# PKU-Alignment/SafeVLA

Measured on AMD Instinct MI355X. Metric: env-steps/sec through PPO-Lagrangian update, higher is better.
Workload: dtype bf16

## Files before the change

### safevla_amd/csrc/attn_q1.hip

```cpp
#include "attn_common.h"

#define Q1_D 512
#define Q1_H 8
#define Q1_WAVES 8
#define Q1_THREADS (Q1_WAVES * 64)
#define Q1_SMAX 256
#define Q1_SLOTS (Q1_SMAX / Q1_WAVES)
#define Q1_RED_FLOATS (Q1_H * Q1_D)
#define Q1_LDS_FWD ((size_t)(Q1_SMAX * Q1_H + 4 * Q1_RED_FLOATS) * sizeof(float))
#define Q1_LDS_BWD ((size_t)(2 * Q1_SMAX * Q1_H + 4 * Q1_RED_FLOATS) * sizeof(float))

__device__ __forceinline__ void q1_unpack(bf16x8 v, float (&f)[8]) {
    const u32x4 w = __builtin_bit_cast(u32x4, v);
#pragma unroll
    for (int i = 0; i < 4; ++i) { f[2 * i] = bf_lo(w[i]); f[2 * i + 1] = bf_hi(w[i]); }
}

__device__ __forceinline__ void q1_token_head_products(const bf16_t* __restrict__ X, const bf16_t* __restrict__ V, int S, float mul, float* out, int w, int lane) {
    constexpr int NT = Q1_SMAX / (16 * Q1_WAVES), NK = Q1_D / 32;
    const int ql = lane & 15, g = lane >> 4;
    const bf16_t* vb = V + (size_t)(ql & (Q1_H - 1)) * Q1_D + 8 * g;
    bf16x8 a[NT][NK], b[NK];
#pragma unroll
    for (int tt = 0; tt < NT; ++tt) {
        const bf16_t* xa = X + (size_t)min((w + Q1_WAVES * tt) * 16 + ql, S - 1) * Q1_D + 8 * g;
#pragma unroll
        for (int kk = 0; kk < NK; ++kk) a[tt][kk] = *(const bf16x8*)(xa + kk * 32);
    }
#pragma unroll
    for (int kk = 0; kk < NK; ++kk) b[kk] = *(const bf16x8*)(vb + kk * 32);
#pragma unroll
    for (int tt = 0; tt < NT; ++tt) {
        const int j0 = (w + Q1_WAVES * tt) * 16;
        f32x4 acc = {0.f, 0.f, 0.f, 0.f};
#pragma unroll
        for (int kk = 0; kk < NK; ++kk) acc = mfma16(a[tt][kk], b[kk], acc);
        if (ql < Q1_H) {
#pragma unroll
            for (int i = 0; i < 4; ++i) {
                const int j = j0 + 4 * g + i;
                if (j < S) out[j * Q1_H + ql] = acc[i] * mul;
            }
        }
    }
}

__device__ __forceinline__ void q1_load_slices(const bf16_t* __restrict__ X, int S, int w, int lane, bf16x8 (&xr)[Q1_SLOTS]) {
#pragma unroll
    for (int t = 0; t < Q1_SLOTS; ++t) {
        const int j = min(w + Q1_WAVES * t, S - 1);
        xr[t] = *(const bf16x8*)(X + (size_t)j * Q1_D + lane * 8);
    }
}

__device__ __forceinline__ void q1_token_sums(const bf16x8 (&xr)[Q1_SLOTS], const float* coef, int S, int w, float (&acc)[Q1_H][8]) {
#pragma unroll
    for (int h = 0; h < Q1_H; ++h)
#pragma unroll
        for (int e = 0; e < 8; ++e) acc[h][e] = 0.f;
#pragma unroll
    for (int t = 0; t < Q1_SLOTS; ++t) {
        const int j = w + Q1_WAVES * t;
        if (j < S) {
            const f32x4 c0 = *(const f32x4*)(coef + j * Q1_H), c1 = *(const f32x4*)(coef + j * Q1_H + 4);
            float x[8];
            q1_unpack(xr[t], x);
#pragma unroll
            for (int h = 0; h < 4; ++h)
#pragma unroll
                for (int e = 0; e < 8; ++e) { acc[h][e] += c0[h] * x[e]; acc[h + 4][e] += c1[h] * x[e]; }
        }
    }
}

__device__ __forceinline__ void q1_red_store(const float (&acc)[Q1_H][8], float* buf, int lane) {
#pragma unroll
    for (int h = 0; h < Q1_H; ++h) {
        *(f32x4*)(buf + h * Q1_D + lane * 8) = f32x4{acc[h][0], acc[h][1], acc[h][2], acc[h][3]};
        *(f32x4*)(buf + h * Q1_D + lane * 8 + 4) = f32x4{acc[h][4], acc[h][5], acc[h][6], acc[h][7]};
    }
}
__device__ __forceinline__ void q1_red_add(float (&acc)[Q1_H][8], const float* buf, int lane) {
#pragma unroll
    for (int h = 0; h < Q1_H; ++h) {
        const f32x4 a = *(const f32x4*)(buf + h * Q1_D + lane * 8), b = *(const f32x4*)(buf + h * Q1_D + lane * 8 + 4);
#pragma unroll
        for (int e = 0; e < 4; ++e) { acc[h][e] += a[e]; acc[h][e + 4] += b[e]; }
    }
}
__device__ __forceinline__ void q1_reduce_write(float (&acc)[Q1_H][8], float* red, int w, int lane, bf16_t* __restrict__ out) {
    if (w >= 4) q1_red_store(acc, red + (w - 4) * Q1_RED_FLOATS, lane);
    __syncthreads();
    if (w < 4) q1_red_add(acc, red + w * Q1_RED_FLOATS, lane);
    if (w == 2 || w == 3) q1_red_store(acc, red + w * Q1_RED_FLOATS, lane);
    __syncthreads();
    if (w < 2) q1_red_add(acc, red + (w + 2) * Q1_RED_FLOATS, lane);
    if (w == 1) q1_red_store(acc, red + Q1_RED_FLOATS, lane);
    __syncthreads();
    if (w == 0) {
        q1_red_add(acc, red + Q1_RED_FLOATS, lane);
#pragma unroll
        for (int h = 0; h < Q1_H; ++h) *(bf16x8*)(out + h * Q1_D + lane * 8) = pack8(acc[h]);
    }
}

struct Q1Args {
    const bf16_t* X; long ldx;
    const bf16_t* QT;
    bf16_t* C; float* SIG; float* P;
    const bf16_t* DC; const float* DSIG;
    bf16_t* DX; long lddx; bf16_t* DQT;
    int S; float scale; DropCfg drop;
};

__global__ void __launch_bounds__(Q1_THREADS, 1) attn_q1_fwd_kernel(Q1Args p) {
    extern __shared__ __attribute__((aligned(16))) char smem[];
    float* sc = (float*)smem;
    float* red = sc + Q1_SMAX * Q1_H;
    const int w = __builtin_amdgcn_readfirstlane(threadIdx.x >> 6), lane = threadIdx.x & 63, S = p.S;
    const size_t r = blockIdx.x;
    const DropCfg drop = drop_resolve(p.drop);
    const bf16_t* X = p.X + r * p.ldx;
    q1_token_head_products(X, p.QT + r * (Q1_H * Q1_D), S, p.scale, sc, w, lane);
    bf16x8 xr[Q1_SLOTS];
    q1_load_slices(X, S, w, lane, xr);
    __syncthreads();
    {
        const int h = w;
        float v[Q1_SMAX / 64], m = -INFINITY, sum = 0.f, sig = 0.f;
#pragma unroll
        for (int i = 0; i < Q1_SMAX / 64; ++i) {
            const int j = lane + 64 * i;
            v[i] = j < S ? sc[j * Q1_H + h] : -INFINITY;
            m = fmaxf(m, v[i]);
        }
        m = wave_max(m);
#pragma unroll
        for (int i = 0; i < Q1_SMAX / 64; ++i) { v[i] = __expf(v[i] - m); sum += v[i]; }
        const float inv = 1.f / wave_sum(sum);
        const unsigned long long e0 = att_drop_row(S, Q1_H, (int)r, h, 0);
#pragma unroll
        for (int i = 0; i < Q1_SMAX / 64; ++i) {
            const int j = lane + 64 * i;
            if (j < S) {
                const float pr = v[i] * inv;
                const float pd = (!drop.thr || att_keep1(drop, e0 + j)) ? pr * drop.scale : 0.f;
                p.P[(r * Q1_H + h) * S + j] = pr;
                sc[j * Q1_H + h] = pd;
                sig += pd;
            }
        }
        sig = wave_sum(sig);
        if (lane == 0) p.SIG[r * Q1_H + h] = sig;
    }
    __syncthreads();
    float acc[Q1_H][8];
    q1_token_sums(xr, sc, S, w, acc);
    q1_reduce_write(acc, red, w, lane, p.C + r * (Q1_H * Q1_D));
}

__global__ void __launch_bounds__(Q1_THREADS, 1) attn_q1_bwd_kernel(Q1Args p) {
    extern __shared__ __attribute__((aligned(16))) char smem[];
    float* dsb = (float*)smem;
    float* pdb = dsb + Q1_SMAX * Q1_H;
    float* red = pdb + Q1_SMAX * Q1_H;
    const int w = __builtin_amdgcn_readfirstlane(threadIdx.x >> 6), lane = threadIdx.x & 63, S = p.S;
    const size_t r = blockIdx.x;
    const DropCfg drop = drop_resolve(p.drop);
    const bf16_t* X = p.X + r * p.ldx;
    q1_token_head_products(X, p.DC + r * (Q1_H * Q1_D), S, 1.f, dsb, w, lane);
    bf16x8 xr[Q1_SLOTS];
    q1_load_slices(X, S, w, lane, xr);
    __syncthreads();
    {
        const int h = w;
        const float dsig = p.DSIG[r * Q1_H + h];
        const unsigned long long e0 = att_drop_row(S, Q1_H, (int)r, h, 0);
        float pr[Q1_SMAX / 64], dp[Q1_SMAX / 64], delta = 0.f;
#pragma unroll
        for (int i = 0; i < Q1_SMAX / 64; ++i) {
            const int j = lane + 64 * i;
            pr[i] = 0.f; dp[i] = 0.f;
            if (j < S) {
                pr[i] = p.P[(r * Q1_H + h) * S + j];
                const bool keep = !drop.thr || att_keep1(drop, e0 + j);
                dp[i] = keep ? (dsb[j * Q1_H + h] + dsig) * drop.scale : 0.f;
                pdb[j * Q1_H + h] = keep ? pr[i] * drop.scale : 0.f;
                delta += pr[i] * dp[i];
            }
        }
        delta = wave_sum(delta);
#pragma unroll
        for (int i = 0; i < Q1_SMAX / 64; ++i) {
            const int j = lane + 64 * i;
            if (j < S) dsb[j * Q1_H + h] = p.scale * pr[i] * (dp[i] - delta);
        }
    }
    __syncthreads();
    {
        float acc[Q1_H][8];
        q1_token_sums(xr, dsb, S, w, acc);
        q1_reduce_write(acc, red, w, lane, p.DQT + r * (Q1_H * Q1_D));
    }
    float qf[Q1_H][8], cf[Q1_H][8];
    const bf16_t* QT = p.QT + r * (Q1_H * Q1_D) + lane * 8;
    const bf16_t* DC = p.DC + r * (Q1_H * Q1_D) + lane * 8;
#pragma unroll
    for (int h = 0; h < Q1_H; ++h) {
        q1_unpack(*(const bf16x8*)(QT + h * Q1_D), qf[h]);
        q1_unpack(*(const bf16x8*)(DC + h * Q1_D), cf[h]);
    }
    bf16_t* DX = p.DX + r * p.lddx;
#pragma unroll 1
    for (int j = w; j < S; j += Q1_WAVES) {
        const f32x4 s0 = *(const f32x4*)(dsb + j * Q1_H), s1 = *(const f32x4*)(dsb + j * Q1_H + 4);
        const f32x4 d0 = *(const f32x4*)(pdb + j * Q1_H), d1 = *(const f32x4*)(pdb + j * Q1_H + 4);
        float o[8];
#pragma unroll
        for (int e = 0; e < 8; ++e) o[e] = 0.f;
#pragma unroll
        for (int h = 0; h < 4; ++h)
#pragma unroll
            for (int e = 0; e < 8; ++e) {
                o[e] += s0[h] * qf[h][e] + d0[h] * cf[h][e];
                o[e] += s1[h] * qf[h + 4][e] + d1[h] * cf[h + 4][e];
            }
        *(bf16x8*)(DX + (size_t)j * Q1_D + lane * 8) = pack8(o);
    }
}

static bool q1_shape_ok(int R, int S, long ldx) { return R > 0 && S > 0 && S <= Q1_SMAX && ldx >= (long)S * Q1_D && ldx % 8 == 0; }

extern "C" int svla_attn_q1_fwd_bf16(const bf16_t* X, long ldx, const bf16_t* QT, bf16_t* C, float* SIG, float* P, int R, int S, float scale,
                                     const svla_dropout* drop, void* stream) {
    if (!X || !QT || !C || !SIG || !P || !q1_shape_ok(R, S, ldx)) return SVLA_EINVAL;
    Q1Args p{};
    p.X = X; p.ldx = ldx; p.QT = QT; p.C = C; p.SIG = SIG; p.P = P; p.S = S; p.scale = scale; p.drop = drop_cfg(drop);
    return svla_launch<attn_q1_fwd_kernel>(dim3(R), dim3(Q1_THREADS), Q1_LDS_FWD, (hipStream_t)stream, p);
}

extern "C" int svla_attn_q1_bwd_bf16(const bf16_t* X, long ldx, const bf16_t* QT, const bf16_t* DC, const float* DSIG, const float* P,
                                     bf16_t* DX, long lddx, bf16_t* DQT, int R, int S, float scale, const svla_dropout* drop, void* stream) {
    if (!X || !QT || !DC || !DSIG || !P || !DX || !DQT || !q1_shape_ok(R, S, ldx) || !q1_shape_ok(R, S, lddx)) return SVLA_EINVAL;
    Q1Args p{};
    p.X = X; p.ldx = ldx; p.QT = QT; p.DC = DC; p.DSIG = DSIG; p.P = (float*)P; p.DX = DX; p.lddx = lddx; p.DQT = DQT;
    p.S = S; p.scale = scale; p.drop = drop_cfg(drop);
    return svla_launch<attn_q1_bwd_kernel>(dim3(R), dim3(Q1_THREADS), Q1_LDS_BWD, (hipStream_t)stream, p);
}

__global__ void __launch_bounds__(256) head_expand_kernel(const bf16_t* __restrict__ v, long ldv, int R, bf16_t* __restrict__ E, const float* __restrict__ bias,
                                                          float* __restrict__ dot, const float* __restrict__ sigma, bf16_t* __restrict__ vs) {
    const size_t r = (size_t)blockIdx.x * 4 + (threadIdx.x >> 6);
    const int lane = threadIdx.x & 63, hl = lane >> 3;
    if (r >= (size_t)R) return;
    const bf16x8 x = *(const bf16x8*)(v + r * ldv + lane * 8);
    const bf16x8 z = {0, 0, 0, 0, 0, 0, 0, 0};
#pragma unroll
    for (int h = 0; h < Q1_H; ++h) *(bf16x8*)(E + (r * Q1_H + h) * Q1_D + lane * 8) = h == hl ? x : z;
    if (!bias && !sigma) return;
    float f[8];
    q1_unpack(x, f);
    if (bias) {
        float s = 0.f;
#pragma unroll
        for (int e = 0; e < 8; ++e) s += f[e] * bias[lane * 8 + e];
        s += __shfl_xor(s, 1, 64); s += __shfl_xor(s, 2, 64); s += __shfl_xor(s, 4, 64);
        if ((lane & 7) == 0) dot[r * Q1_H + hl] = s;
    }
    if (sigma) {
        const float sg = sigma[r * Q1_H + hl];
#pragma unroll
        for (int e = 0; e < 8; ++e) f[e] *= sg;
        *(bf16x8*)(vs + r * Q1_D + lane * 8) = pack8(f);
    }
}
__global__ void __launch_bounds__(256) head_pick_kernel(const bf16_t* __restrict__ G, int R, const float* __restrict__ sigma, const float* __restrict__ bias,
                                                        bf16_t* __restrict__ out, long ldo) {
    const size_t r = (size_t)blockIdx.x * 4 + (threadIdx.x >> 6);
    const int lane = threadIdx.x & 63, hl = lane >> 3;
    if (r >= (size_t)R) return;
    bf16x8 x = *(const bf16x8*)(G + (r * Q1_H + hl) * Q1_D + lane * 8);
    if (sigma) {
        float f[8];
        q1_unpack(x, f);
        const float sg = sigma[r * Q1_H + hl];
#pragma unroll
        for (int e = 0; e < 8; ++e) f[e] += sg * bias[lane * 8 + e];
        x = pack8(f);
    }
    *(bf16x8*)(out + r * ldo + lane * 8) = x;
}

extern "C" int svla_head_expand_bf16(const bf16_t* v, long ldv, int R, bf16_t* E, const float* bias, float* dot, const float* sigma, bf16_t* vs, void* stream) {
    if (!v || !E || R <= 0 || ldv < Q1_D || ldv % 8 || (bias && !dot) || (sigma && !vs)) return SVLA_EINVAL;
    hipLaunchKernelGGL(head_expand_kernel, dim3((R + 3) / 4), dim3(256), 0, (hipStream_t)stream, v, ldv, R, E, bias, dot, sigma, vs);
    return svla_launch_status();
}
extern "C" int svla_head_pick_bf16(const bf16_t* G, int R, const float* sigma, const float* bias, bf16_t* out, long ldo, void* stream) {
    if (!G || !out || R <= 0 || ldo < Q1_D || ldo % 8 || (sigma && !bias)) return SVLA_EINVAL;
    hipLaunchKernelGGL(head_pick_kernel, dim3((R + 3) / 4), dim3(256), 0, (hipStream_t)stream, G, R, sigma, bias, out, ldo);
    return svla_launch_status();
}
```

Measured before the change: 8030.

## Add persistent register-resident streaming kernels for single-query attention fwd/bwd

Adds new persistent forward and backward kernels for single-query cross-attention, made the default path; the old two-pass kernels stay behind an environment variable. Each workgroup holds a row's tokens in registers, computes scores with MFMA from a swizzled LDS image, and prefetches the next row's X, QT and DC while finishing the current row. Grid size is capped at the CU count. The aim is to read X once per row instead of twice and to hide global load latency. In exchange it uses heavy register and LDS pressure at one workgroup per CU, and occupancy is lower.

```diff
diff --git a/safevla_amd/csrc/attn_q1.hip b/safevla_amd/csrc/attn_q1.hip
--- a/safevla_amd/csrc/attn_q1.hip
+++ b/safevla_amd/csrc/attn_q1.hip
@@ -1,3 +1,4 @@
+#include <stdlib.h>
 #include "attn_common.h"
 
 #define Q1_D 512
@@ -231,9 +232,18 @@
 
 static bool q1_shape_ok(int R, int S, long ldx) { return R > 0 && S > 0 && S <= Q1_SMAX && ldx >= (long)S * Q1_D && ldx % 8 == 0; }
 
+int svla_q1_stream_fwd(const bf16_t* X, long ldx, const bf16_t* QT, bf16_t* C, float* SIG, float* P, int R, int S, float scale, DropCfg drop, hipStream_t stream);
+int svla_q1_stream_bwd(const bf16_t* X, long ldx, const bf16_t* QT, const bf16_t* DC, const float* DSIG, const float* P, bf16_t* DX, long lddx, bf16_t* DQT,
+                       int R, int S, float scale, DropCfg drop, hipStream_t stream);
+static bool q1_two_pass() {
+    static const bool on = [] { const char* e = getenv("SVLA_Q1_TWO_PASS"); return e && *e && strcmp(e, "0") != 0; }();
+    return on;
+}
+
 extern "C" int svla_attn_q1_fwd_bf16(const bf16_t* X, long ldx, const bf16_t* QT, bf16_t* C, float* SIG, float* P, int R, int S, float scale,
                                      const svla_dropout* drop, void* stream) {
     if (!X || !QT || !C || !SIG || !P || !q1_shape_ok(R, S, ldx)) return SVLA_EINVAL;
+    if (!q1_two_pass()) return svla_q1_stream_fwd(X, ldx, QT, C, SIG, P, R, S, scale, drop_cfg(drop), (hipStream_t)stream);
     Q1Args p{};
     p.X = X; p.ldx = ldx; p.QT = QT; p.C = C; p.SIG = SIG; p.P = P; p.S = S; p.scale = scale; p.drop = drop_cfg(drop);
     return svla_launch<attn_q1_fwd_kernel>(dim3(R), dim3(Q1_THREADS), Q1_LDS_FWD, (hipStream_t)stream, p);
@@ -242,6 +252,7 @@
 extern "C" int svla_attn_q1_bwd_bf16(const bf16_t* X, long ldx, const bf16_t* QT, const bf16_t* DC, const float* DSIG, const float* P,
                                      bf16_t* DX, long lddx, bf16_t* DQT, int R, int S, float scale, const svla_dropout* drop, void* stream) {
     if (!X || !QT || !DC || !DSIG || !P || !DX || !DQT || !q1_shape_ok(R, S, ldx) || !q1_shape_ok(R, S, lddx)) return SVLA_EINVAL;
+    if (!q1_two_pass()) return svla_q1_stream_bwd(X, ldx, QT, DC, DSIG, P, DX, lddx, DQT, R, S, scale, drop_cfg(drop), (hipStream_t)stream);
     Q1Args p{};
     p.X = X; p.ldx = ldx; p.QT = QT; p.DC = DC; p.DSIG = DSIG; p.P = (float*)P; p.DX = DX; p.lddx = lddx; p.DQT = DQT;
     p.S = S; p.scale = scale; p.drop = drop_cfg(drop);
diff --git a/safevla_amd/csrc/attn_q1_stream.hip b/safevla_amd/csrc/attn_q1_stream.hip
--- /dev/null
+++ b/safevla_amd/csrc/attn_q1_stream.hip
@@ -0,0 +1,301 @@
+#include "attn_common.h"
+
+#define QS_D 512
+#define QS_H 8
+#define QS_WAVES 8
+#define QS_THREADS (QS_WAVES * 64)
+#define QS_SMAX 256
+#define QS_SLOTS (QS_SMAX / QS_WAVES)
+#define QS_TILE_ELEMS (16 * QS_D)
+#define QS_STAGE_BYTES ((size_t)QS_WAVES * QS_TILE_ELEMS * sizeof(bf16_t))
+#define QS_RED_FLOATS (QS_H * QS_D)
+#define QS_COEF_FLOATS (QS_SMAX * QS_H)
+#define QS_VTAB_BYTES ((size_t)QS_H * QS_D * sizeof(bf16_t))
+#define QS_LDS_FWD (QS_STAGE_BYTES + (size_t)QS_COEF_FLOATS * sizeof(float) + QS_VTAB_BYTES)
+#define QS_LDS_BWD (QS_STAGE_BYTES + (size_t)2 * QS_COEF_FLOATS * sizeof(float) + 2 * QS_VTAB_BYTES)
+static_assert(QS_WAVES * QS_RED_FLOATS * sizeof(float) <= QS_STAGE_BYTES, "the 8 partials alias the staging images");
+static_assert(QS_LDS_BWD <= 160 * 1024, "one workgroup's LDS");
+
+struct Q1SArgs {
+    const bf16_t* X; long ldx;
+    const bf16_t* QT;
+    bf16_t* C; float* SIG; float* P;
+    const bf16_t* DC; const float* DSIG;
+    bf16_t* DX; long lddx; bf16_t* DQT;
+    int R, S; float scale; DropCfg drop;
+};
+
+#define QS_FRESH(w_, lane_, S_) asm volatile("" : "+s"(w_), "+v"(lane_), "+s"(S_))
+
+__device__ __forceinline__ void qs_unpack(bf16x8 v, float (&f)[8]) {
+    const u32x4 w = __builtin_bit_cast(u32x4, v);
+#pragma unroll
+    for (int i = 0; i < 4; ++i) { f[2 * i] = bf_lo(w[i]); f[2 * i + 1] = bf_hi(w[i]); }
+}
+
+__device__ __forceinline__ int qs_tile0(int w, int tt) { return (w + QS_WAVES * tt) * 16; }
+
+__device__ __forceinline__ void qs_load_row(const bf16_t* __restrict__ X, int S, int w, int lane, bf16x8 (&xr)[QS_SLOTS]) {
+#pragma unroll
+    for (int t = 0; t < QS_SLOTS; ++t) {
+        const int j = min(qs_tile0(w, t >> 4) + (t & 15), S - 1);
+        xr[t] = *(const bf16x8*)(X + (size_t)j * QS_D + lane * 8);
+    }
+}
+__device__ __forceinline__ void qs_vtab_put(bf16_t* vtab, int w, int lane, bf16x8 v) {
+    asm volatile("" : "+s"(w), "+v"(lane));
+    *(bf16x8*)(vtab + w * QS_D + ((lane ^ (2 * w)) << 3)) = v;
+}
+
+template <int TT> __device__ __forceinline__ void qs_tile_products(const bf16x8 (&xr)[QS_SLOTS], const bf16_t* vtab, bf16_t* img, int S, float mul, float* out,
+                                                                   int w, int lane) {
+    const int ql = lane & 15, g = lane >> 4, hh = lane & (QS_H - 1);
+#pragma unroll
+    for (int i = 0; i < 16; ++i) *(bf16x8*)(img + i * QS_D + ((lane ^ i) << 3)) = xr[16 * TT + i];
+    f32x4 acc = {0.f, 0.f, 0.f, 0.f};
+#pragma unroll
+    for (int kk = 0; kk < QS_D / 32; ++kk)
+        acc = mfma16(*(const bf16x8*)(img + ql * QS_D + (((4 * kk + g) ^ ql) << 3)), *(const bf16x8*)(vtab + hh * QS_D + (((4 * kk + g) ^ (2 * hh)) << 3)), acc);
+    if (ql < QS_H) {
+#pragma unroll
+        for (int i = 0; i < 4; ++i) {
+            const int j = qs_tile0(w, TT) + 4 * g + i;
+            if (j < S) out[j * QS_H + ql] = acc[i] * mul;
+        }
+    }
+}
+__device__ __forceinline__ void qs_products(const bf16x8 (&xr)[QS_SLOTS], const bf16_t* vtab, bf16_t* img, int S, float mul, float* out, int w, int lane) {
+    QS_FRESH(w, lane, S);
+    if (qs_tile0(w, 0) < S) qs_tile_products<0>(xr, vtab, img, S, mul, out, w, lane);
+    if (qs_tile0(w, 1) < S) qs_tile_products<1>(xr, vtab, img, S, mul, out, w, lane);
+}
+
+__device__ __forceinline__ void qs_token_sums_refill(bf16x8 (&xr)[QS_SLOTS], const float* coef, int S, int w, int lane, const bf16_t* __restrict__ Xn,
+                                                     float (&acc)[QS_H][8]) {
+    QS_FRESH(w, lane, S);
+#pragma unroll
+    for (int h = 0; h < QS_H; ++h)
+#pragma unroll
+        for (int e = 0; e < 8; ++e) acc[h][e] = 0.f;
+#pragma unroll
+    for (int t = 0; t < QS_SLOTS; ++t) {
+        const int j = qs_tile0(w, t >> 4) + (t & 15);
+        if (j < S) {
+            const f32x4 c0 = *(const f32x4*)(coef + j * QS_H), c1 = *(const f32x4*)(coef + j * QS_H + 4);
+            float x[8];
+            qs_unpack(xr[t], x);
+#pragma unroll
+            for (int h = 0; h < 4; ++h)
+#pragma unroll
+                for (int e = 0; e < 8; ++e) { acc[h][e] += c0[h] * x[e]; acc[h + 4][e] += c1[h] * x[e]; }
+        }
+        xr[t] = *(const bf16x8*)(Xn + (size_t)min(j, S - 1) * QS_D + lane * 8);
+    }
+}
+
+__device__ __forceinline__ void qs_red_put(const float (&acc)[QS_H][8], float* red, int w, int lane) {
+    asm volatile("" : "+s"(w), "+v"(lane));
+#pragma unroll
+    for (int h = 0; h < QS_H; ++h) {
+        *(f32x4*)(red + w * QS_RED_FLOATS + h * QS_D + lane * 4) = f32x4{acc[h][0], acc[h][1], acc[h][2], acc[h][3]};
+        *(f32x4*)(red + w * QS_RED_FLOATS + h * QS_D + 256 + lane * 4) = f32x4{acc[h][4], acc[h][5], acc[h][6], acc[h][7]};
+    }
+}
+__device__ __forceinline__ void qs_head_sum_write(const float* red, int w, int lane, bf16_t* __restrict__ out) {
+    asm volatile("" : "+s"(w), "+v"(lane));
+    float s[8] = {0.f, 0.f, 0.f, 0.f, 0.f, 0.f, 0.f, 0.f};
+#pragma unroll
+    for (int v = 0; v < QS_WAVES; ++v) {
+        const f32x4 a = *(const f32x4*)(red + v * QS_RED_FLOATS + w * QS_D + lane * 4), b = *(const f32x4*)(red + v * QS_RED_FLOATS + w * QS_D + 256 + lane * 4);
+#pragma unroll
+        for (int e = 0; e < 4; ++e) { s[e] += a[e]; s[e + 4] += b[e]; }
+    }
+    *(bf16x8*)(out + w * QS_D + lane * 8) = pack8(s);
+}
+
+__global__ void __launch_bounds__(QS_THREADS, 1) attn_q1_stream_fwd_kernel(Q1SArgs p) {
+    extern __shared__ __attribute__((aligned(16))) char smem[];
+    bf16_t* stage = (bf16_t*)smem;
+    float* red = (float*)smem;
+    float* sc = (float*)(smem + QS_STAGE_BYTES);
+    bf16_t* vtab = (bf16_t*)(sc + QS_COEF_FLOATS);
+    const int w = __builtin_amdgcn_readfirstlane(threadIdx.x >> 6), lane = threadIdx.x & 63, S = p.S;
+    const DropCfg drop = drop_resolve(p.drop);
+    bf16_t* img = stage + w * QS_TILE_ELEMS;
+    size_t r = blockIdx.x;
+    bf16x8 xr[QS_SLOTS];
+    qs_load_row(p.X + r * p.ldx, S, w, lane, xr);
+    qs_vtab_put(vtab, w, lane, *(const bf16x8*)(p.QT + r * (QS_H * QS_D) + threadIdx.x * 8));
+    __syncthreads();
+    for (;;) {
+        const size_t rn = r + gridDim.x;
+        const bool more = rn < (size_t)p.R;
+        const size_t rl = more ? rn : r;
+        int tid = threadIdx.x;
+        asm volatile("" : "+v"(tid));
+        const bf16x8 vq = *(const bf16x8*)(p.QT + rl * (QS_H * QS_D) + tid * 8);
+        qs_products(xr, vtab, img, S, p.scale, sc, w, lane);
+        __syncthreads();
+        qs_vtab_put(vtab, w, lane, vq);
+        {
+            const int h = w;
+            float v[QS_SMAX / 64], m = -INFINITY, sum = 0.f, sig = 0.f;
+#pragma unroll
+            for (int i = 0; i < QS_SMAX / 64; ++i) {
+                const int j = lane + 64 * i;
+                v[i] = j < S ? sc[j * QS_H + h] : -INFINITY;
+                m = fmaxf(m, v[i]);
+            }
+            m = wave_max(m);
+#pragma unroll
+            for (int i = 0; i < QS_SMAX / 64; ++i) { v[i] = __expf(v[i] - m); sum += v[i]; }
+            const float inv = 1.f / wave_sum(sum);
+            const unsigned long long e0 = att_drop_row(S, QS_H, (int)r, h, 0);
+#pragma unroll
+            for (int i = 0; i < QS_SMAX / 64; ++i) {
+                const int j = lane + 64 * i;
+                if (j < S) {
+                    const float pr = v[i] * inv;
+                    const float pd = (!drop.thr || att_keep1(drop, e0 + j)) ? pr * drop.scale : 0.f;
+                    p.P[(r * QS_H + h) * S + j] = pr;
+                    sc[j * QS_H + h] = pd;
+                    sig += pd;
+                }
+            }
+            sig = wave_sum(sig);
+            if (lane == 0) p.SIG[r * QS_H + h] = sig;
+        }
+        __syncthreads();
+        float acc[QS_H][8];
+        qs_token_sums_refill(xr, sc, S, w, lane, p.X + rl * p.ldx, acc);
+        qs_red_put(acc, red, w, lane);
+        __syncthreads();
+        qs_head_sum_write(red, w, lane, p.C + r * (QS_H * QS_D));
+        if (!more) break;
+        r = rn;
+        __syncthreads();
+    }
+}
+
+__global__ void __launch_bounds__(QS_THREADS, 1) attn_q1_stream_bwd_kernel(Q1SArgs p) {
+    extern __shared__ __attribute__((aligned(16))) char smem[];
+    bf16_t* stage = (bf16_t*)smem;
+    float* red = (float*)smem;
+    float* dsb = (float*)(smem + QS_STAGE_BYTES);
+    float* pdb = dsb + QS_COEF_FLOATS;
+    bf16_t* vdc = (bf16_t*)(pdb + QS_COEF_FLOATS);
+    bf16_t* vqt = vdc + QS_H * QS_D;
+    const int w = __builtin_amdgcn_readfirstlane(threadIdx.x >> 6), lane = threadIdx.x & 63, S = p.S;
+    const DropCfg drop = drop_resolve(p.drop);
+    bf16_t* img = stage + w * QS_TILE_ELEMS;
+    size_t r = blockIdx.x;
+    bf16x8 xr[QS_SLOTS];
+    qs_load_row(p.X + r * p.ldx, S, w, lane, xr);
+    float pr[QS_SMAX / 64], dsig;
+#pragma unroll
+    for (int i = 0; i < QS_SMAX / 64; ++i) {
+        const int j = lane + 64 * i;
+        pr[i] = p.P[(r * QS_H + w) * S + min(j, S - 1)];
+    }
+    dsig = p.DSIG[r * QS_H + w];
+    qs_vtab_put(vdc, w, lane, *(const bf16x8*)(p.DC + r * (QS_H * QS_D) + threadIdx.x * 8));
+    qs_vtab_put(vqt, w, lane, *(const bf16x8*)(p.QT + r * (QS_H * QS_D) + threadIdx.x * 8));
+    __syncthreads();
+    for (;;) {
+        const size_t rn = r + gridDim.x;
+        const bool more = rn < (size_t)p.R;
+        const size_t rl = more ? rn : r;
+        int tid = threadIdx.x;
+        asm volatile("" : "+v"(tid));
+        const bf16x8 vd = *(const bf16x8*)(p.DC + rl * (QS_H * QS_D) + tid * 8);
+        const bf16x8 vq = *(const bf16x8*)(p.QT + rl * (QS_H * QS_D) + tid * 8);
+        qs_products(xr, vdc, img, S, 1.f, dsb, w, lane);
+        __syncthreads();
+        {
+            int h = w, lv = lane, Sv = S;
+            QS_FRESH(h, lv, Sv);
+            const unsigned long long e0 = att_drop_row(Sv, QS_H, (int)r, h, 0);
+            float dp[QS_SMAX / 64], delta = 0.f;
+#pragma unroll
+            for (int i = 0; i < QS_SMAX / 64; ++i) {
+                const int j = lv + 64 * i;
+                dp[i] = 0.f;
+                if (j < Sv) {
+                    const bool keep = !drop.thr || att_keep1(drop, e0 + j);
+                    dp[i] = keep ? (dsb[j * QS_H + h] + dsig) * drop.scale : 0.f;
+                    pdb[j * QS_H + h] = keep ? pr[i] * drop.scale : 0.f;
+                    delta += pr[i] * dp[i];
+                }
+            }
+            delta = wave_sum(delta);
+#pragma unroll
+            for (int i = 0; i < QS_SMAX / 64; ++i) {
+                const int j = lv + 64 * i;
+                if (j < Sv) dsb[j * QS_H + h] = p.scale * pr[i] * (dp[i] - delta);
+            }
+#pragma unroll
+            for (int i = 0; i < QS_SMAX / 64; ++i) {
+                const int j = lv + 64 * i;
+                pr[i] = p.P[(rl * QS_H + h) * Sv + min(j, Sv - 1)];
+            }
+            dsig = p.DSIG[rl * QS_H + w];
+        }
+        __syncthreads();
+        {
+            float qf[QS_H][4], cf[QS_H][4];
+            int wv = w, lv = lane, Sv = S;
+            QS_FRESH(wv, lv, Sv);
+            const int half = wv >> 2;
+#pragma unroll
+            for (int h = 0; h < QS_H; ++h) {
+                const int off = h * QS_D + (((32 * half + (lv >> 1)) ^ (2 * h)) << 3) + 4 * (lv & 1);
+                const u32x2 q = *(const u32x2*)(vqt + off), c = *(const u32x2*)(vdc + off);
+                qf[h][0] = bf_lo(q[0]); qf[h][1] = bf_hi(q[0]); qf[h][2] = bf_lo(q[1]); qf[h][3] = bf_hi(q[1]);
+                cf[h][0] = bf_lo(c[0]); cf[h][1] = bf_hi(c[0]); cf[h][2] = bf_lo(c[1]); cf[h][3] = bf_hi(c[1]);
+            }
+            bf16_t* DX = p.DX + r * p.lddx + 256 * half + 4 * lv;
+#pragma unroll 2
+            for (int j = wv & 3; j < Sv; j += 4) {
+                const f32x4 s0 = *(const f32x4*)(dsb + j * QS_H), s1 = *(const f32x4*)(dsb + j * QS_H + 4);
+                const f32x4 d0 = *(const f32x4*)(pdb + j * QS_H), d1 = *(const f32x4*)(pdb + j * QS_H + 4);
+                float o[4] = {0.f, 0.f, 0.f, 0.f};
+#pragma unroll
+                for (int h = 0; h < 4; ++h)
+#pragma unroll
+                    for (int e = 0; e < 4; ++e) {
+                        o[e] += s0[h] * qf[h][e] + d0[h] * cf[h][e];
+                        o[e] += s1[h] * qf[h + 4][e] + d1[h] * cf[h + 4][e];
+                    }
+                *(u32x2*)(DX + (size_t)j * QS_D) = u32x2{pack_bf2(o[0], o[1]), pack_bf2(o[2], o[3])};
+            }
+        }
+        __builtin_amdgcn_sched_barrier(0);
+        {
+            float acc[QS_H][8];
+            qs_token_sums_refill(xr, dsb, S, w, lane, p.X + rl * p.ldx, acc);
+            qs_red_put(acc, red, w, lane);
+        }
+        __syncthreads();
+        qs_head_sum_write(red, w, lane, p.DQT + r * (QS_H * QS_D));
+        qs_vtab_put(vdc, w, lane, vd);
+        qs_vtab_put(vqt, w, lane, vq);
+        if (!more) break;
+        r = rn;
+        __syncthreads();
+    }
+}
+
+static int qs_grid(int R) { const int cu = svla_cu_count(); return cu > 0 && cu < R ? cu : R; }
+
+int svla_q1_stream_fwd(const bf16_t* X, long ldx, const bf16_t* QT, bf16_t* C, float* SIG, float* P, int R, int S, float scale, DropCfg drop, hipStream_t stream) {
+    Q1SArgs p{};
+    p.X = X; p.ldx = ldx; p.QT = QT; p.C = C; p.SIG = SIG; p.P = P; p.R = R; p.S = S; p.scale = scale; p.drop = drop;
+    return svla_launch<attn_q1_stream_fwd_kernel>(dim3(qs_grid(R)), dim3(QS_THREADS), QS_LDS_FWD, stream, p);
+}
+int svla_q1_stream_bwd(const bf16_t* X, long ldx, const bf16_t* QT, const bf16_t* DC, const float* DSIG, const float* P, bf16_t* DX, long lddx, bf16_t* DQT,
+                       int R, int S, float scale, DropCfg drop, hipStream_t stream) {
+    Q1SArgs p{};
+    p.X = X; p.ldx = ldx; p.QT = QT; p.DC = DC; p.DSIG = DSIG; p.P = (float*)P; p.DX = DX; p.lddx = lddx; p.DQT = DQT;
+    p.R = R; p.S = S; p.scale = scale; p.drop = drop;
+    return svla_launch<attn_q1_stream_bwd_kernel>(dim3(qs_grid(R)), dim3(QS_THREADS), QS_LDS_BWD, stream, p);
+}
```

After: 8087, median of 6. Within noise of the previous version (+0.7%).
